# ming71/rotate-yolov3

Hardware: AMD Instinct MI355X
Metric: images/sec fwd+bwd at 608^2 (train step, backend=hip) (higher is better)
Workload: dtype bf16; 1 GPU; configs[3]: Darknet-53 train step (fwd + riou loss + bwd + grad all-reduce + SGD), bs=64/GPU 608x608, synthetic HRSC-shaped targets; global_batch=64, parallelism=dp1, gradients=250 MB fp32 in 4 flat buckets, fp32 on the wire

## Files before the change

include/ryolo.h:

```cpp
#ifndef RYOLO_H
#define RYOLO_H

#include <stddef.h>
#include <stdint.h>

#ifdef __cplusplus
extern "C" {
#endif

#define RYOLO_OK 0
#define RYOLO_EINVAL -1
#define RYOLO_ELAUNCH -2
#define RYOLO_ETOOBIG -3

#define RYOLO_RNMS_MAX_BOXES 262144

const char *ryolo_strerror(int code);
int ryolo_abi_version(void);
const char *ryolo_build_id(void);
int ryolo_set_tuning(const char *name, const char *value);

size_t ryolo_rnms_workspace_bytes(int n);
int ryolo_rnms(const float *dets, int n, int row_stride, float thr, int64_t *keep_out, int32_t *num_keep,
               void *workspace, size_t workspace_bytes, void *stream);
// ... 97 lines not shown
int ryolo_yolo_decode(const void *head, int head_cstride, int bs, int ny, int nx, int na, int no,
                      const float *anchors, float stride, float context_factor, int arc, float *io,
                      long long io_rows_per_image, long long io_row_offset, float *p, void *stream);

int ryolo_conv_head_decode_supported(const ryolo_conv_desc *desc, int na, int no);
int ryolo_conv_head_decode(const ryolo_conv_desc *desc, const void *x, const void *w_packed, const float *scale, const float *shift,
                           const float *anchors, int na, int no, float stride, float context_factor, int arc, float *io,
                           long long io_rows_per_image, long long io_row_offset, float *p, void *stream);
int ryolo_conv_head_decode_store(const ryolo_conv_desc *desc, const void *x, const void *w_packed, const float *scale, const float *shift,
                                 int na, int no, void *head, int head_cstride, float *p, void *stream);

int ryolo_add_nhwc(const void *a, int a_cstride, const void *b, int b_cstride, void *y, int y_cstride,
                   long long npix, int C, void *stream);
int ryolo_upsample_nhwc(const void *x, int x_cstride, void *y, int y_cstride, int N, int H, int W, int C, int scale,
                        void *stream);
int ryolo_maxpool_nhwc(const void *x, int x_cstride, void *y, int y_cstride, int N, int H, int W, int C, int ksize,
                       int stride, void *stream);

size_t ryolo_se_workspace_bytes(int N, int H, int W, int C);
int ryolo_se_nhwc(const void *x, int x_cstride, const float *w1 , const float *w2 ,
                  int hidden, void *y, int y_cstride, int N, int H, int W, int C,
                  float *gate_out , void *workspace, size_t workspace_bytes, void *stream);
size_t ryolo_se_bwd_workspace_bytes(int N, int H, int W, int C, int hidden);
int ryolo_se_bwd_nhwc(const void *x, int x_cstride, const void *dy, int dy_cstride, const float *w1 ,
                      const float *w2 , int hidden, void *dx , int dx_cstride, int dx_accumulate,
                      float *dw1, float *dw2 , int accumulate_w, int N, int H, int W, int C,
                      float *gate_out , void *workspace, size_t workspace_bytes, void *stream);


int ryolo_conv0_recompute_supported(const ryolo_conv_desc *desc);
int ryolo_conv0_bn_act_fwd(const ryolo_conv_desc *desc, const void *x, const void *w_packed, const float *scale, const float *shift,
                           int act, const float *slope, void *y, void *stream);
size_t ryolo_conv0_bn_bwd_workspace_bytes(void);
int ryolo_conv0_bn_bwd(const ryolo_conv_desc *desc, const void *x, const void *w_packed, const void *dy, int dy_cstride,
                       const float *scale, const float *shift, const float *mean, const float *invstd, int act, const float *slope,
                       void *dz, int dz_cstride, float *dgamma, float *dbeta, float *dslope, void *workspace, size_t workspace_bytes,
                       int workspace_is_zero, void *stream);
size_t ryolo_conv0_bn_bwd_wgrad_workspace_bytes(void);
int ryolo_conv0_bn_bwd_wgrad(const ryolo_conv_desc *desc, const void *x, const void *w_packed, const void *dy, int dy_cstride,
                             const float *scale, const float *shift, const float *mean, const float *invstd, int act, const float *slope,
                             float *dgamma, float *dbeta, float *dslope, float *grad_oihw, int cin_real, int accumulate, void *workspace,
                             size_t workspace_bytes, void *stream);
int ryolo_conv_stat_rows(const ryolo_conv_desc *desc);
int ryolo_conv2d_bn_act_stats(const ryolo_conv_desc *desc, const void *x, const void *w_packed, const float *scale,
                              const float *shift, const void *residual, void *y,
                              double *stat_part ,
                              void *stream);
int ryolo_bn_finalize(double *stat_part, int rows, int cpad, int C, long long count, float eps, float momentum,
                      const float *gamma, const float *beta, float *mean, float *invstd, float *scale, float *shift,
                      float *running_mean , float *running_var, void *stream);
int ryolo_bn_act_fwd(const void *z, int z_cstride, const float *scale, const float *shift, int act,
                     const float *slope , const void *residual, int res_cstride, void *y,
                     int y_cstride, long long npix, int C, void *stream);
size_t ryolo_bn_act_bwd_workspace_bytes(long long npix, int C);
int ryolo_bn_act_bwd(const void *z, int z_cstride, const void *dy, int dy_cstride, const float *scale, const float *shift,
                     const float *mean, const float *invstd, int act, const float *slope, void *dz, int dz_cstride,
                     long long npix, int C, float *dgamma, float *dbeta, float *dslope, void *workspace,
                     size_t workspace_bytes, void *stream);
size_t ryolo_conv_packed_dgrad_bytes(int Cout, int Cin, int ksize, int stride);
int ryolo_conv_dgrad_tap_table(int ksize, int stride, int *host_out );
int ryolo_conv_pack_weights_dgrad(const float *w_oihw, int Cout, int Cin, int ksize, int stride, void *packed,
                                  const int *taps_table ,
                                  void *stream);
int ryolo_conv2d_dgrad(const ryolo_conv_desc *forward_desc, const void *dz, int dz_cstride, const void *packed_dgrad,
                       const float *ones, const float *zeros , void *dx, int accumulate, void *stream);
int ryolo_conv2d_dgrad_bnreduce_rows(const ryolo_conv_desc *forward_desc);
int ryolo_conv2d_dgrad_bnreduce(const ryolo_conv_desc *forward_desc, const void *dz, int dz_cstride, const void *packed_dgrad,
                                const float *ones, const float *zeros, void *dx, int accumulate,
                                const void *z , int z_cstride,
                                const float *scale, const float *shift, const float *mean, const float *invstd ,
                                const float *slope , float *part , void *stream);
int ryolo_bn_act_bwd_reduced(const void *z, int z_cstride, const void *dy, int dy_cstride, const float *scale, const float *shift,
                             const float *mean, const float *invstd, int act , const float *slope, void *dz,
                             int dz_cstride, long long npix, int C, float *dgamma, float *dbeta, float *dslope, const float *part,
                             int rows, void *workspace , size_t workspace_bytes, void *stream);
size_t ryolo_conv_wgrad_workspace_bytes(const ryolo_conv_desc *forward_desc);
int ryolo_conv2d_wgrad_partials(const ryolo_conv_desc *forward_desc, const void *x, const void *dz, int dz_cstride, int Cin_real,
                                float *grad_oihw, int accumulate, void *workspace, size_t workspace_bytes, void *stream);
int ryolo_conv2d_wgrad_reduce(const ryolo_conv_desc *forward_desc, const void *x, const void *dz, int dz_cstride, int Cin_real,
                              float *grad_oihw, int accumulate, void *workspace, size_t workspace_bytes, void *stream);

typedef struct ryolo_wgrad_reduce_job {
    const float *part;
    float *g;
    int S, Cout, Cin_real, Cin_k, ks, Kpad, Cout_pad, accumulate;
    int kind;
    int block_begin, block_end;
    int wide;
} ryolo_wgrad_reduce_job;
int ryolo_conv_wgrad_reduce_job_fill(ryolo_wgrad_reduce_job *host_job, const ryolo_conv_desc *forward_desc, int Cin_real, const void *workspace,
                                     float *grad_oihw, int accumulate);
int ryolo_conv_wgrad_reduce_batch(const ryolo_wgrad_reduce_job *device_jobs, int njobs, int total_blocks, void *stream);
int ryolo_conv2d_wgrad(const ryolo_conv_desc *forward_desc, const void *x, const void *dz, int dz_cstride, int Cin_real,
                       float *grad_oihw , int accumulate, void *workspace,
                       size_t workspace_bytes, void *stream);
int ryolo_upsample2x_bwd(const void *dy, int dy_cstride, void *dx, int dx_cstride, int N, int H, int W, int C,
                         int accumulate, void *stream);
int ryolo_pgrad_to_nhwc(const float *pgrad, int bs, int na, int ny, int nx, int no, void *out, int out_cstride,
                        void *stream);

typedef struct ryolo_pack_job {
    const void *src;
    void *dst;
    int kind, Cout, Cin, KS, Cin_pad, ntaps, Kpad, rows;
    int khs[9], kws[9];
    int block_begin, block_end;
// ... 78 lines not shown
```

rotate-yolov3_amd/csrc/train.hip:

```cpp
#include "conv_common.h"

using namespace ryolo_detail;

namespace {

__global__ void __launch_bounds__(1024) bn_finalize_kernel(double *__restrict__ part, int R, int cpad, int C, float count, float eps,
                                   float momentum, const float *__restrict__ gamma, const float *__restrict__ beta,
                                   float *__restrict__ mean, float *__restrict__ invstd, float *__restrict__ scale,
                                   float *__restrict__ shift, float *__restrict__ run_mean, float *__restrict__ run_var) {
    __shared__ double red[2][32][33];
    const int cx = threadIdx.x & 31, ry = threadIdx.x >> 5;
    const int c = blockIdx.x * 32 + cx;
    double s = 0.0, q = 0.0;
    if (c < C) {
        for (int r0 = ry; r0 < R; r0 += 32 * 8) {
            double a[8], b[8];
#pragma unroll
            for (int u = 0; u < 8; u++) {
                const int r = r0 + 32 * u;
                a[u] = r < R ? part[(size_t)r * 2 * cpad + c] : 0.0;
                b[u] = r < R ? part[(size_t)r * 2 * cpad + cpad + c] : 0.0;
            }
#pragma unroll
            for (int u = 0; u < 8; u++) {
// ... 37 lines not shown
    const float n = (1.f + e) * (1.f + e);
    const float t = (n - 1.f) / (n + 1.f);
    return t + x * (1.f - t * t) * (e / (1.f + e));
}

constexpr long long NT_MIN_BYTES = 128ll << 20;
#ifdef RYOLO_MP_ABLATION
static int g_nt[3] = {-1, -1, -1};
inline bool nt_pass(int kind, long long npix, int C) { return g_nt[kind] < 0 ? npix * C * 2 >= NT_MIN_BYTES : g_nt[kind] != 0; }
#else
inline bool nt_pass(int, long long npix, int C) { return npix * C * 2 >= NT_MIN_BYTES; }
#endif
template <bool NTL>
__device__ __forceinline__ bf16x8 ld8(const __bf16 *p) {
    if constexpr (NTL) return __builtin_nontemporal_load((const bf16x8 *)p);
    else return *(const bf16x8 *)p;
}
template <bool NTL>
__device__ __forceinline__ void st8(__bf16 *p, const bf16x8 &v) {
    if constexpr (NTL) __builtin_nontemporal_store(v, (bf16x8 *)p);
    else *(bf16x8 *)p = v;
}

template <int ACT, bool NTL = false>
__global__ void bn_act_fwd_kernel(const __bf16 *__restrict__ z, int z_cs, const float *__restrict__ scale,
                                  const float *__restrict__ shift, const float *__restrict__ slope_p,
                                  const __bf16 *__restrict__ res, int res_cs, __bf16 *__restrict__ y, int y_cs,
                                  long long npix, int C) {
    const int cpr = C / 8;
    const long long total = npix * cpr;
    const float slope = slope_p ? slope_p[0] : 0.f;
    for (long long i = (long long)blockIdx.x * blockDim.x + threadIdx.x; i < total;
         i += (long long)gridDim.x * blockDim.x) {
        const long long pix = i / cpr;
        const int c = (int)(i % cpr) * 8;
        const bf16x8 v = ld8<NTL>(z + pix * z_cs + c);
        bf16x8 o;
#pragma unroll
        for (int e = 0; e < 8; e++) {
            float u = (float)v[e] * scale[c + e] + shift[c + e];
            if (ACT == 1) u = u > 0.f ? u : u * slope;
            else if (ACT == 2) u = mish_f(u);
            o[e] = (__bf16)u;
        }
        if (res) {
            const bf16x8 r = ld8<NTL>(res + pix * res_cs + c);
#pragma unroll
            for (int e = 0; e < 8; e++) o[e] = (__bf16)((float)o[e] + (float)r[e]);
        }
        st8<NTL>(y + pix * y_cs + c, o);
    }
}

constexpr int BWD_SLAB_MIN = 128;
#ifdef RYOLO_MP_ABLATION
static int g_bwd_slabs = 1024, g_bwd_slab_min = BWD_SLAB_MIN;
inline long long bwd_slab(long long npix) {
    long long s = (npix + g_bwd_slabs - 1) / g_bwd_slabs;
    return s < g_bwd_slab_min ? g_bwd_slab_min : s;
}
#else
inline long long bwd_slab(long long npix) {
    const long long s = (npix + 1023) / 1024;
    return s < BWD_SLAB_MIN ? BWD_SLAB_MIN : s;
}
#endif
template <int ACT, bool NTL = false>
__global__ void __launch_bounds__(256)
bn_act_bwd_reduce_kernel(const __bf16 *__restrict__ z, int z_cs, const __bf16 *__restrict__ dy, int dy_cs,
                         const float *__restrict__ scale, const float *__restrict__ shift,
                         const float *__restrict__ mean, const float *__restrict__ invstd,
                         const float *__restrict__ slope_p, long long npix, int C, int CT, float *__restrict__ part, long long SL) {
    __shared__ float red[256][25];
    const int cl = threadIdx.x % CT, pl = threadIdx.x / CT, npl = 256 / CT;
    const int c = (blockIdx.x * CT + cl) * 8;
    const int slab = blockIdx.y;
    const long long p0 = (long long)slab * SL;
    const long long p1 = p0 + SL < npix ? p0 + SL : npix;
    const float slope = slope_p ? slope_p[0] : 0.f;
    float s1[8], s2[8], s3[8];
#pragma unroll
    for (int e = 0; e < 8; e++) s1[e] = s2[e] = s3[e] = 0.f;
    if (c < C) {
        float sc[8], sh[8], mu[8], is[8];
#pragma unroll
        for (int e = 0; e < 8; e++) {
            sc[e] = scale ? scale[c + e] : 1.f; sh[e] = scale ? shift[c + e] : 0.f;
            mu[e] = scale ? mean[c + e] : 0.f; is[e] = scale ? invstd[c + e] : 0.f;
        }
        auto accum = [&](const bf16x8 &zv, const bf16x8 &gv) {
#pragma unroll
            for (int e = 0; e < 8; e++) {
                const float zf = (float)zv[e], d = (float)gv[e];
                float g = d;
                if (scale) {
                    const float u = zf * sc[e] + sh[e];
                    if (ACT == 1 && u <= 0.f) { g = d * slope; s3[e] += d * u; }
                    else if (ACT == 2) g = d * mish_grad(u);
                    s2[e] += g * (zf - mu[e]);
                }
                s1[e] += g;
            }
        };
        long long pix = p0 + pl;
        for (; pix + 3 * npl < p1; pix += 4 * npl) {
            bf16x8 zv[4], gv[4];
// ... 253 lines not shown
__global__ void __launch_bounds__(256) pgrad_to_nhwc_tiled_kernel(const float *__restrict__ g, int na, int plane, int no,
                                                                  __bf16 *__restrict__ out, int out_cs, int npix) {
    extern __shared__ __attribute__((aligned(16))) __bf16 pg_lds[];
    const int C = na * no;
    const int p0 = blockIdx.x * PG_PIX;
    const int per_a = PG_PIX * no;
    for (int idx = threadIdx.x; idx < na * per_a; idx += 256) {
        const int a = idx / per_a, rem = idx - a * per_a;
        const int pl = rem / no, k = rem - pl * no;
        const int gp = p0 + pl;
        if (gp < npix) {
            const int n = gp / plane, pp = gp - n * plane;
            pg_lds[pl * C + a * no + k] = (__bf16)g[((size_t)(n * na + a) * plane + pp) * no + k];
        }
    }
    __syncthreads();
    const int cpr = C / 8;
    for (int idx = threadIdx.x; idx < PG_PIX * cpr; idx += 256) {
        const int pl = idx / cpr, c = (idx - pl * cpr) * 8;
        if (p0 + pl < npix) *(bf16x8 *)(out + (size_t)(p0 + pl) * out_cs + c) = *(const bf16x8 *)(pg_lds + pl * C + c);
    }
}

constexpr int ELEM_BLOCKS = 4096;
inline int ok_launch() { return hipGetLastError() == hipSuccess ? RYOLO_OK : RYOLO_ELAUNCH; }

}

extern "C" {

int ryolo_bn_finalize(double *stat_part, int rows, int cpad, int C, long long count, float eps, float momentum,
                      const float *gamma, const float *beta, float *mean, float *invstd, float *scale, float *shift,
                      float *running_mean, float *running_var, void *stream) {
    if (!stat_part || !gamma || !beta || !mean || !invstd || !scale || !shift || rows <= 0 || C <= 0 || count <= 0)
        return RYOLO_EINVAL;
    hipLaunchKernelGGL(bn_finalize_kernel, dim3((C + 31) / 32), dim3(1024), 0, (hipStream_t)stream, stat_part, rows, cpad, C,
                       (float)count, eps, momentum, gamma, beta, mean, invstd, scale, shift, running_mean, running_var);
    return ok_launch();
}

int ryolo_bn_act_fwd(const void *z, int z_cstride, const float *scale, const float *shift, int act, const float *slope,
                     const void *residual, int res_cstride, void *y, int y_cstride, long long npix, int C, void *stream) {
    if (!z || !scale || !shift || !y || npix <= 0 || C <= 0 || (C & 7) || (z_cstride & 7) || (y_cstride & 7))
        return RYOLO_EINVAL;
    if (act < 0 || act > 2) return RYOLO_EINVAL;
    const bool ntl = nt_pass(0, npix, C);
#define RYOLO_BN_FWD(A)                                                                                                   \
    hipLaunchKernelGGL((ntl ? bn_act_fwd_kernel<A, true> : bn_act_fwd_kernel<A, false>), dim3(grid_for(npix * (C / 8))), dim3(256), 0, (hipStream_t)stream,           \
                       (const __bf16 *)z, z_cstride, scale, shift, slope, (const __bf16 *)residual, res_cstride,          \
                       (__bf16 *)y, y_cstride, npix, C)
    if (act == 0) RYOLO_BN_FWD(0); else if (act == 1) RYOLO_BN_FWD(1); else RYOLO_BN_FWD(2);
#undef RYOLO_BN_FWD
    return ok_launch();
}

size_t ryolo_bn_act_bwd_workspace_bytes(long long npix, int C) {
    const long long nslab = (npix + bwd_slab(npix) - 1) / bwd_slab(npix);
    return (size_t)nslab * 3 * C * 4 + (size_t)3 * C * 4;
}

static int bn_act_bwd_impl(const void *z, int z_cstride, const void *dy, int dy_cstride, const float *scale, const float *shift,
                           const float *mean, const float *invstd, int act, const float *slope, void *dz, int dz_cstride,
                           long long npix, int C, float *dgamma, float *dbeta, float *dslope, void *workspace,
                           size_t workspace_bytes, const float *pre_part, int pre_rows, void *stream_);

int ryolo_bn_act_bwd(const void *z, int z_cstride, const void *dy, int dy_cstride, const float *scale, const float *shift,
                     const float *mean, const float *invstd, int act, const float *slope, void *dz, int dz_cstride,
                     long long npix, int C, float *dgamma, float *dbeta, float *dslope, void *workspace,
                     size_t workspace_bytes, void *stream_) {
    return bn_act_bwd_impl(z, z_cstride, dy, dy_cstride, scale, shift, mean, invstd, act, slope, dz, dz_cstride, npix, C, dgamma, dbeta,
                           dslope, workspace, workspace_bytes, nullptr, 0, stream_);
}

int ryolo_bn_act_bwd_reduced(const void *z, int z_cstride, const void *dy, int dy_cstride, const float *scale, const float *shift,
                             const float *mean, const float *invstd, int act, const float *slope, void *dz, int dz_cstride,
                             long long npix, int C, float *dgamma, float *dbeta, float *dslope, const float *part, int rows,
                             void *workspace, size_t workspace_bytes, void *stream_) {
    if (!part || rows <= 0 || !scale || act != 1) return RYOLO_EINVAL;
    return bn_act_bwd_impl(z, z_cstride, dy, dy_cstride, scale, shift, mean, invstd, act, slope, dz, dz_cstride, npix, C, dgamma, dbeta,
                           dslope, workspace, workspace_bytes, part, rows, stream_);
}

static int bn_act_bwd_impl(const void *z, int z_cstride, const void *dy, int dy_cstride, const float *scale, const float *shift,
                           const float *mean, const float *invstd, int act, const float *slope, void *dz, int dz_cstride,
                           long long npix, int C, float *dgamma, float *dbeta, float *dslope, void *workspace,
                           size_t workspace_bytes, const float *pre_part, int pre_rows, void *stream_) {
    if (!z || !dy || npix <= 0 || C <= 0 || (C & 7) || (z_cstride & 7) || (dy_cstride & 7) || !workspace) return RYOLO_EINVAL;
    if (workspace_bytes < (pre_part ? (size_t)3 * C * 4 : ryolo_bn_act_bwd_workspace_bytes(npix, C))) return RYOLO_EINVAL;
    if (scale && (!shift || !mean || !invstd || !dz || (dz_cstride & 7))) return RYOLO_EINVAL;
    hipStream_t stream = (hipStream_t)stream_;
    int nslab = pre_part ? pre_rows : (int)((npix + bwd_slab(npix) - 1) / bwd_slab(npix));
    float *part = pre_part ? const_cast<float *>(pre_part) : (float *)workspace;
    float *s1 = pre_part ? (float *)workspace : part + (size_t)nslab * 3 * C, *s2 = s1 + C, *s3 = s2 + C;
    if (pre_part && pre_rows >= BWD_FOLD_MIN_ROWS && workspace_bytes >= (size_t)(3 + 3 * BWD_FOLD) * C * 4) {
        float *folded = s3 + C;
        const int per = (pre_rows + BWD_FOLD - 1) / BWD_FOLD;
        hipLaunchKernelGGL(bn_act_bwd_fold_kernel, dim3((C + 31) / 32, BWD_FOLD), dim3(1024), 0, stream, part, pre_rows, C, per, folded);
        part = folded;
        nslab = (pre_rows + per - 1) / per;
    }
    float *dsl = (scale && act == 1) ? dslope : nullptr;
    int CT = 32;
    while (CT > 1 && CT > C / 8) CT >>= 1;
    if (act < 0 || act > 2) return RYOLO_EINVAL;
    const bool nt_red = nt_pass(1, npix, C), nt_app = nt_pass(2, npix, C);
#define RYOLO_BN_REDK(A) (nt_red ? bn_act_bwd_reduce_kernel<A, true> : bn_act_bwd_reduce_kernel<A, false>)
// ... 84 lines not shown
```

rotate-yolov3_amd/model/hip_train_ops.py:

```python
import ctypes as C

import torch

from .. import _lib
from .._lib import PackJob, WgradReduceJob
from . import hip_ops
from .hip_ops import ConvDesc, _check_nhwc, cpad, pack_weights

ARC_FOCAL, ARC_UBCE, ARC_UCE = 1, 2, 4


def arc_flags(arc):
    f = ARC_FOCAL if 'F' in arc else 0
    if 'default' in arc:
        return f
    if 'BCE' in arc:
        return f | ARC_UBCE
    if 'CE' in arc:
        return f | ARC_UCE
    raise ValueError("unknown arc %r" % (arc,))


class WgradReduceBatch(object):

# ... 126 lines not shown


def conv0_bn_bwd_wgrad_ws(device):
    return torch.empty(_lib.lib().ryolo_conv0_bn_bwd_wgrad_workspace_bytes(), dtype=torch.uint8, device=device)


def conv0_bn_bwd_wgrad(d, x, packed_w, dy, stats, act, slope, dgamma, dbeta, dslope, grad_w, cin_real, accumulate, ws):
    mean, invstd, scale, shift = stats
    _lib.check(_lib.lib().ryolo_conv0_bn_bwd_wgrad(C.byref(d), x.data_ptr(), packed_w.data_ptr(), dy.data_ptr(), dy.stride(2),
                                                   scale.data_ptr(), shift.data_ptr(), mean.data_ptr(), invstd.data_ptr(), act,
                                                   slope.data_ptr() if slope is not None else None, dgamma.data_ptr(), dbeta.data_ptr(),
                                                   dslope.data_ptr() if dslope is not None else None, grad_w.data_ptr(), int(cin_real),
                                                   1 if accumulate else 0, ws.data_ptr(), ws.numel(), _s(x.device)), "ryolo_conv0_bn_bwd_wgrad")


def conv_fwd_plain(d, x, packed_w, ones, shift, z):
    d.out_cstride = _check_nhwc(z, "z")
    _lib.check(_lib.lib().ryolo_conv2d_bn_act(C.byref(d), x.data_ptr(), packed_w.data_ptr(), ones.data_ptr(), shift.data_ptr(),
                                              None, z.data_ptr(), _s(x.device)), "ryolo_conv2d_bn_act")


def conv_head_decode_store(hf, x, packed_w, ones, shift, head, p):
    d = ConvDesc(*hf['desc'])
    d.in_cstride = _check_nhwc(x, "x")
    hcs = _check_nhwc(head, "head")
    if not p.is_contiguous() or p.dtype != torch.float32:
        raise ValueError("conv_head_decode_store: p must be contiguous fp32")
    _lib.check(_lib.lib().ryolo_conv_head_decode_store(C.byref(d), x.data_ptr(), packed_w.data_ptr(), ones.data_ptr(), shift.data_ptr(),
                                                       hf['na'], hf['no'], head.data_ptr(), hcs, p.data_ptr(), _s(x.device)),
               "ryolo_conv_head_decode_store")


def bn_finalize(part, C_, count, gamma, beta, eps=1e-5, momentum=0.1, running_mean=None, running_var=None, out=None):
    dev = part.device
    if out is None:
        out = [torch.empty(C_, dtype=torch.float32, device=dev) for _ in range(4)]
    _lib.check(_lib.lib().ryolo_bn_finalize(part.data_ptr(), part.shape[0], part.shape[2], C_, int(count), eps, momentum,
                                            gamma.data_ptr(), beta.data_ptr(), out[0].data_ptr(), out[1].data_ptr(),
                                            out[2].data_ptr(), out[3].data_ptr(),
                                            running_mean.data_ptr() if running_mean is not None else None,
                                            running_var.data_ptr() if running_var is not None else None, _s(dev)),
               "ryolo_bn_finalize")
    return out


def bn_act_fwd(z, scale, shift, act, slope, y, residual=None):
    n, h, w, c = z.shape
    _lib.check(_lib.lib().ryolo_bn_act_fwd(z.data_ptr(), z.stride(2), scale.data_ptr(), shift.data_ptr(), act,
                                           slope.data_ptr() if slope is not None else None,
                                           residual.data_ptr() if residual is not None else None,
                                           residual.stride(2) if residual is not None else 0, y.data_ptr(), y.stride(2),
                                           n * h * w, c, _s(z.device)), "ryolo_bn_act_fwd")
    return y


def bn_act_bwd(z, dy, stats, act, slope, dz, dgamma, dbeta, dslope, ws):
    n, h, w, c = z.shape
    mean, invstd, scale, shift = stats if stats is not None else (None, None, None, None)
    p = lambda t: t.data_ptr() if t is not None else None
    _lib.check(_lib.lib().ryolo_bn_act_bwd(z.data_ptr(), z.stride(2), dy.data_ptr(), dy.stride(2), p(scale), p(shift), p(mean),
                                           p(invstd), act, p(slope), p(dz), dz.stride(2) if dz is not None else 0,
                                           n * h * w, c, p(dgamma), p(dbeta), p(dslope), ws.data_ptr(), ws.numel(),
                                           _s(z.device)), "ryolo_bn_act_bwd")


def bn_bwd_ws_bytes(npix, c):
    return _lib.lib().ryolo_bn_act_bwd_workspace_bytes(npix, c)


_tap_tables = {}


def dgrad_tap_table(ksize, stride, device):
    key = (ksize, stride, device.index)
    t = _tap_tables.get(key)
    if t is None:
        host = (C.c_int * 72)()
        _lib.check(_lib.lib().ryolo_conv_dgrad_tap_table(ksize, stride, host), "ryolo_conv_dgrad_tap_table")
        t = torch.tensor(list(host), dtype=torch.int32, device=device)
        _tap_tables[key] = t
    return t


def pack_weights_dgrad(weight, stride, out=None):
    cout, cin, k, _ = weight.shape
    L = _lib.lib()
    nbytes = L.ryolo_conv_packed_dgrad_bytes(cout, cin, k, stride)
    if out is None:
        out = torch.empty(nbytes, dtype=torch.uint8, device=weight.device)
    w = weight.contiguous()
    table = dgrad_tap_table(k, stride, weight.device)
    _lib.check(L.ryolo_conv_pack_weights_dgrad(w.data_ptr(), cout, cin, k, stride, out.data_ptr(), table.data_ptr(),
                                               _s(weight.device)), "ryolo_conv_pack_weights_dgrad")
    return out


def conv_dgrad(d, dz, packed_dgrad, ones, zeros, dx, accumulate):
    _lib.check(_lib.lib().ryolo_conv2d_dgrad(C.byref(d), dz.data_ptr(), dz.stride(2), packed_dgrad.data_ptr(), ones.data_ptr(),
                                             zeros.data_ptr(), dx.data_ptr(), 1 if accumulate else 0, _s(dz.device)),
               "ryolo_conv2d_dgrad")


def dgrad_bnreduce_rows(d):
    return _lib.lib().ryolo_conv2d_dgrad_bnreduce_rows(C.byref(d))


# ... 338 lines not shown
```

rotate-yolov3_amd/model/plan.py:

```python
import ctypes as C
from collections import namedtuple

from .. import _lib
from .._lib import ACT_LINEAR, ConvDesc

View = namedtuple('View', 'buf off C H W cs')
EvalPlan = namedtuple('EvalPlan', 'shapes buffers x views ops')
CONV_TYPES = ('convolutional', 'd-convolutional')
TrainPlan = namedtuple('TrainPlan', 'shapes buffers x act grd forward blocks backward')


class Refused(RuntimeError):
    """the configuration is refused at plan time (as opposed to a bug in the planner)"""


def _abs(i, l):
    return l if l > 0 else i + l


def _sources(i, d):
    return [_abs(i, int(v)) for v in d['layers'].split(',')]


def shared_attrs(d):
# ... 304 lines not shown
            recompute = bool(i == 0 and cv['bn'] and i not in conv_res and conv0_recompute
                             and _query('ryolo_conv0_recompute_supported', desc))
            head_fused = None
            if (head_decode and yolos is not None and i + 1 < n and defs[i + 1]['type'] == 'yolo' and readers[i] == [i + 1] and i not in home
                    and i not in conv_res and not cv['bn'] and cv['k'] == 1 and cv['s'] == 1 and c % 8 == 0):
                na, no = yolos[i + 1]
                ht = (N, xin.H, xin.W, xin.C, c, 1, 1, 0, xin.cs, c, 0, ACT_LINEAR, 0.0, 1, 0)
                if _query('ryolo_conv_head_decode_supported', ht, int(na), int(no)):
                    head_fused = dict(desc=ht, na=int(na), no=int(no))
            blk = dict(layer=i, desc=desc, xin=xin, xin_g=xin_g, y=y, dy=dy, res=act[conv_res[i]] if i in conv_res else None,
                       res_g=grd[conv_res[i]] if i in conv_res else None, res_alias=res_alias, bn=cv['bn'], act=cv['act'], shape=shp[i],
                       recompute=recompute, one_pass=bool(recompute and xin_g is None and conv0_one_pass), head_fused=head_fused)
            blocks.append(blk)
            forward.append(('conv', i, blk))
        elif t == 'shortcut':
            a, b = i - 1, _abs(i, int(d['from']))
            act[i], grd[i] = pair_for(i)
            forward.append(('add', i, (act[a], act[b], act[i], grd[a], grd[b], grd[i])))
        elif t == 'upsample':
            act[i], grd[i] = pair_for(i)
            forward.append(('up', i, (act[i - 1], act[i], grd[i - 1], grd[i])))
        elif t == 'route':
            if i in alias:
                act[i], grd[i] = act[alias[i]], grd[alias[i]]
        elif t == 'yolo':
            act[i], grd[i] = act[i - 1], grd[i - 1]
            forward.append(('yolo', i, (act[i], grd[i])))

    init = set()

    def first(g):
        if g in init:
            return False
        init.add(g)
        init.update(children.get(g, ()))
        return True

    heads = [i for kind, i, _ in forward if kind == 'yolo']
    backward = []
    for kind, i, pl in reversed(forward):
        if kind == 'yolo':
            first(pl[1])
            backward.append((kind, i, heads.index(i)))
        elif kind == 'conv':
            res_first = first(pl['res_g']) if (pl['res_g'] is not None and not pl['res_alias']) else None
            backward.append((kind, i, (res_first, first(pl['xin_g']) if pl['xin_g'] is not None else None)))
        elif kind == 'add':
            backward.append((kind, i, (first(pl[3]), first(pl[4]))))
        elif kind == 'up':
            backward.append((kind, i, first(pl[2])))
    return TrainPlan(shp, buffers, x, act, grd, forward, blocks, backward)


def reduce_fusion_pairs(tp):
    by = {b['layer']: b for b in tp.blocks}
    pairs = []
    for (k0, i0, _), (k1, i1, _) in zip(tp.backward[:-1], tp.backward[1:]):
        if k0 != 'conv' or k1 != 'conv':
            continue
        x, y = by[i0], by[i1]
        g, dy = x['xin_g'], y['dy']
        if g is None or not y['bn'] or y['recompute'] or g != dy or dy[2:5] != y['shape'] or g.cs != g.C:
            continue
        rows = _query('ryolo_conv2d_dgrad_bnreduce_rows', x['desc'])
        if rows > 0:
            pairs.append((x, y, rows))
    return pairs
```

rotate-yolov3_amd/model/train_engine.py:

```python
import ctypes as C
import os

import torch
import torch.nn as nn

from .. import _lib
from . import hip_ops as ops
from . import hip_train_ops as tr
from . import plan
from .engine import HipEngine
from .nhwc_batch import NHWC8Batch


class _Fn(torch.autograd.Function):
    @staticmethod
    def forward(ctx, engine, x, anchor):
        ctx.engine = engine
        outs = engine.forward(x)
        return tuple(outs)

    @staticmethod
    def backward(ctx, *grads):
        ctx.engine.backward(grads)
        return None, None, None
# ... 63 lines not shown
                    dz = None if rec['one_pass'] else new_buf(c, h, w)
                else:
                    z, dz = y, dy
                blk = dict(i=i, conv=conv, bn=bn, act=actmod[-1] if actmod else None, mish=any(type(s_).__name__ == 'Mish' for s_ in mods[i]),
                           xin=xin, xin_g=tv(rec['xin_g']), z=z, dz=dz, y=y, dy=dy, desc=desc, res=tv(rec['res']), res_g=tv(rec['res_g']),
                           res_alias=rec['res_alias'], cin_k=xin.shape[-1], k=desc.ksize, s=desc.stride, pad=desc.pad,
                           npix=self.bs * h * w, C=c, recompute=rec['recompute'])
                if rec.get('head_fused') and not actmod and not blk['mish']:
                    blk['head_fused'] = rec['head_fused']
                wgrad_ws = max(wgrad_ws, tr.wgrad_ws_bytes(desc))
                bn_ws = max(bn_ws, tr.bn_bwd_ws_bytes(blk['npix'], c))
                self.blocks.append(blk)
                fwd.append(('conv', i, blk))
            elif kind in ('add', 'up'):
                fwd.append((kind, i, tuple(tv(v) for v in rec)))
            elif kind == 'yolo':
                m = mods[i]
                c, h, w = tp.shapes[i]
                anchors = m.anchors.to(device=device, dtype=torch.float32).contiguous()
                pbuf = torch.empty((self.bs, m.na, h, w, model.nc + 6), dtype=torch.float32, device=device)
                io = None
                if model.nc + 6 > 96 or m.na * (model.nc + 6) > 1024:
                    io = torch.empty((self.bs, m.na * h * w, model.nc + 6), dtype=torch.float32, device=device)
                self.p.append(pbuf)
                hb = self.blocks[-1] if self.blocks and self.blocks[-1]['i'] == i - 1 and self.blocks[-1].get('head_fused') else None
                if hb is not None and (hb['head_fused']['na'], hb['head_fused']['no']) != (m.na, model.nc + 6):
                    hb.pop('head_fused')
                    hb = None
                fwd.append(('yolo', i, (tv(rec[0]), tv(rec[1]), m, anchors, pbuf, io, h, w, hb)))
        self.head_pairs = [(pl[0], pl[1]) for kind, _, pl in fwd if kind == 'yolo']
        self.fused_nhwc = False
        self.head_g_ready = False
        self.head_bias_fold = os.environ.get('RYOLO_HEAD_BIAS_FOLD', '1') != '0'
        self.head_gscale = torch.ones(1, device=device)
        self.head_bias_ready = None
        self._bias_parts = self._bias_ws = None
        self._fold_now = (False,) * len(self.head_pairs)
        self._g_bwd_fold = None
        readers = plan._readers(defs)
        for k, (hd, _) in enumerate(self.head_pairs):
            for b in self.blocks:
                i = b['i']
                if (b['y'] is hd and b['bn'] is None and b['conv'].bias is not None and i + 1 < len(defs) and defs[i + 1]['type'] == 'yolo'
                        and readers[i] == [i + 1]):
                    b['head_k'] = k
        self.batch_reduce = os.environ.get('RYOLO_WGRAD_BATCH_REDUCE', '1') != '0'
        self._wr_batches = {}
        self._ws_w_bytes = max(wgrad_ws, 256)
        self._ws_w = None
        self.ws_b = torch.empty(max(bn_ws, 256), dtype=torch.uint8, device=device)

        self.bplan = [(kind, i, pl, flags) for (kind, i, pl), (_, _, flags) in zip(reversed(fwd), tp.backward)]

    @staticmethod
    def _conv_attrs(m):
        conv = HipEngine._conv_of(m)
        other = [type(s_).__name__ for s_ in m if not isinstance(s_, (nn.Conv2d, nn.BatchNorm2d, nn.PReLU, nn.LeakyReLU))
                 and type(s_).__name__ != 'Mish']
        return dict(cout=conv.out_channels, k=conv.kernel_size[0], s=conv.stride[0], pad=conv.padding[0],
                    bn=HipEngine._bn_of(m) is not None, act=None,
                    refuse="activation %s has no HIP training kernels (use model.backend = 'torch')" % other[0] if other else None)

    def _build_grad_sink(self):
        plist = [q for q in self.model.parameters()]
        views = getattr(self.model, '_dp_grad_views', None)
        ok = views is not None and os.environ.get("RYOLO_DIRECT_GRADS", "1") != "0"
        if ok:
            for q in plist:
                v = views.get(q)
                if (v is None or v.dtype != torch.float32 or not v.is_contiguous() or v.device != q.device or v.shape != q.shape
                        or q.grad is None or q.grad.data_ptr() != v.data_ptr()):
                    ok = False
                    break
        self.direct = bool(ok)
        if ok:
            self.static_flat = None
            self.static_grad = {q: views[q] for q in plist}
        else:
            self.static_flat = torch.zeros(sum(q.numel() for q in plist), dtype=torch.float32, device=self.device)
            off = 0
            for q in plist:
                self.static_grad[q] = self.static_flat[off:off + q.numel()].view_as(q)
                off += q.numel()

    def _reset_grad_sink(self):
        self.static_grad, self.static_flat, self.direct = {}, None, False
        self._segs, self.g_bwd = None, None
        self._wr_batches = {}

    def _check_direct_sink(self):
        if not self.direct:
            return
        rebound = 0
        for q, v in self.static_grad.items():
            g = q.grad
            if g is None:
                v.zero_()
            elif g.data_ptr() != v.data_ptr():
                v.copy_(g)
            else:
                continue
            q.grad = v
            rebound += 1
        if rebound and not getattr(self, '_warned_rebind', False):
            self._warned_rebind = True
            import warnings
# ... 131 lines not shown
                if self.g_fwd is None:
                    self.g_fwd = self._capture(self._forward_launch)
                if self.g_fwd is not None:
                    self.g_fwd.replay()
        return [p for p in self.p]

    def _capture(self, launch):
        dev = self.device
        torch.cuda.synchronize(dev)
        g = torch.cuda.CUDAGraph()
        try:
            with torch.cuda.graph(g, capture_error_mode="thread_local"):
                launch()
            return g
        except Exception as e:
            self.use_graph = False
            self.graph_fallback = "%s: %s" % (type(e).__name__, str(e).splitlines()[0][:200] if str(e) else "")
            import warnings
            warnings.warn("TrainEngine: hipGraph capture failed (%s); continuing with eager launches" % self.graph_fallback)
            try:
                torch.cuda.synchronize(dev)
            except Exception:
                pass
            launch()
            return None

    def _forward_launch(self):
        dev = self.device
        L = _lib.lib()
        if self.nbt is None:
            self.nbt = [pl['bn'].num_batches_tracked for kind, i, pl in self.plan if kind == 'conv' and pl['bn'] is not None]
        if self.nbt:
            torch._foreach_add_(self.nbt, 1)
        if self.packs is None:
            self.packs = tr.WeightPackBatch(dev)
            for kind, i, pl in self.plan:
                if kind != 'conv':
                    continue
                w = pl['conv'].weight
                if w.dtype != torch.float32 or not w.is_contiguous():
                    raise RuntimeError("TrainEngine expects contiguous fp32 conv weights")
                cout, cin, k, _ = w.shape
                pl['packed'] = torch.empty(L.ryolo_conv_packed_weight_bytes(cout, pl['cin_k'], k), dtype=torch.uint8, device=dev)
                pl['packed_d'] = torch.empty(L.ryolo_conv_packed_dgrad_bytes(cout, cin, k, pl['s']), dtype=torch.uint8,
                                             device=dev) if pl['xin_g'] is not None else None
                self.packs.add(w.detach(), pl['s'], pl['cin_k'], pl['packed'], pl['packed_d'])
            self.packs.finalize()
        self.packs.run()
        for kind, i, pl in self.plan:
            if kind == 'conv':
                b = pl
                conv, bn = b['conv'], b['bn']
                if bn is not None:
                    part = tr.conv_fwd_stats(b['desc'], b['xin'], b['packed'], self.ones, self.zeros, b['z'], part=self.stat_part,
                                             clear=False)
                    b['stats'] = tr.bn_finalize(part, b['C'], b['npix'], bn.weight.detach(), bn.bias.detach(), eps=bn.eps,
                                                momentum=bn.momentum, running_mean=bn.running_mean,
                                                running_var=bn.running_var, out=b.get('stats'))
                    slope = b['act'].weight.detach() if isinstance(b['act'], nn.PReLU) else None
                    if isinstance(b['act'], nn.LeakyReLU):
                        if 'leaky' not in b:
                            b['leaky'] = torch.full((1,), b['act'].negative_slope, device=dev)
                        slope = b['leaky']
                    b['slope'] = slope
                    b['actcode'] = 2 if b['mish'] else (1 if slope is not None else 0)
                    if b['recompute']:
                        tr.conv0_bn_act_fwd(b['desc'], b['xin'], b['packed'], b['stats'][2], b['stats'][3], b['actcode'], slope, b['y'])
                    else:
                        tr.bn_act_fwd(b['z'], b['stats'][2], b['stats'][3], b['actcode'], slope, b['y'], residual=b['res'])
                else:
                    if conv.bias is not None:
                        if 'bias_pad' not in b:
                            b['bias_pad'] = torch.zeros(ops.cpad(b['C']), device=dev)
                        b['bias_pad'][:b['C']].copy_(conv.bias.detach())
                        bias = b['bias_pad']
                    else:
                        bias = self.zeros
                    b['bias_now'] = bias
                    if not b.get('head_fused'):
                        tr.conv_fwd_plain(b['desc'], b['xin'], b['packed'], self.ones, bias, b['z'])
                    b['stats'] = None
            elif kind == 'add':
                a, bb, y = pl[0], pl[1], pl[2]
                nn_, hh, ww, cc = y.shape
                _lib.check(L.ryolo_add_nhwc(a.data_ptr(), a.stride(2), bb.data_ptr(), bb.stride(2), y.data_ptr(), y.stride(2),
                                            nn_ * hh * ww, cc, _lib.stream_ptr(dev)), "ryolo_add_nhwc")
            elif kind == 'up':
                xin, y = pl[0], pl[1]
                nn_, hh, ww, cc = xin.shape
                _lib.check(L.ryolo_upsample_nhwc(xin.data_ptr(), xin.stride(2), y.data_ptr(), y.stride(2), nn_, hh, ww, cc, 2,
                                                 _lib.stream_ptr(dev)), "ryolo_upsample_nhwc")
            elif kind == 'yolo':
                head, _, m, anchors, pbuf, io, hh, ww, hb = pl
                stride = float(max(self.H, self.W)) / float(max(hh, ww))
                if hb is not None:
                    tr.conv_head_decode_store(hb['head_fused'], hb['xin'], hb['packed'], self.ones, hb['bias_now'], head, pbuf)
                else:
                    _lib.check(L.ryolo_yolo_decode(head.data_ptr(), head.stride(2), self.bs, hh, ww, m.na, self.model.nc + 6,
                                                   anchors.data_ptr(), stride, 1.0, 0, io.data_ptr() if io is not None else None, m.na * hh * ww, 0,
                                                   pbuf.data_ptr(), _lib.stream_ptr(dev)), "ryolo_yolo_decode")
                if (m.nx, m.ny) != (ww, hh):
                    from .models import create_grids
                    create_grids(m, (self.H, self.W), (ww, hh), dev)

    def backward(self, pgrads):
        dev = self.device
        with torch.cuda.device(dev), torch.no_grad():
            if not hasattr(self, "static_pg"):
                self.static_pg = [torch.zeros_like(p) for p in self.p]
            ready, bias_ready = self.head_g_ready, self.head_bias_ready
            self.head_g_ready, self.head_bias_ready = False, None
            fold = [False] * len(self.static_pg)
            for k, (buf, g) in enumerate(zip(self.static_pg, pgrads)):
                if g is not None and ready and g.data_ptr() == buf.data_ptr():
                    fold[k] = bias_ready is not None and bias_ready[k] is not None
                    continue
                if g is None:
                    buf.zero_()
                elif g.data_ptr() != buf.data_ptr():
                    buf.copy_(g)
# ... 134 lines not shown
```

Measured before the change: 1377 images/s.

## Fuse BN+activation(+residual) forward with the following 1x1 conv and its BN statistics

Adds a persistent kernel that applies BN scale/shift, leaky/PReLU and an optional residual to z, writes y, stages the tile in LDS, and immediately runs the next 1x1 conv (C to C/2) with MFMA. It also accumulates that conv's BN sum and sum-of-squares into stat_part. The engine pairs eligible bn->1x1 conv layers for channel classes 64, 128 and 512, skipping the separate conv_fwd_stats launch and the re-read of y. The cost is more complex register and LDS use, weights held in registers, and a different precision path for the stats, since they are computed from bf16-rounded outputs.

```diff
diff --git a/include/ryolo.h b/include/ryolo.h
--- a/include/ryolo.h
+++ b/include/ryolo.h
@@ -173,6 +173,10 @@
 int ryolo_bn_act_fwd(const void *z, int z_cstride, const float *scale, const float *shift, int act,
                      const float *slope , const void *residual, int res_cstride, void *y,
                      int y_cstride, long long npix, int C, void *stream);
+int ryolo_bn_act_conv1x1_stats_supported(const ryolo_conv_desc *next_1x1, int C, int has_res);
+int ryolo_bn_act_conv1x1_stats(const ryolo_conv_desc *next_1x1, const void *z, int z_cs, const float *scale, const float *shift,
+                               const float *slope, const void *res, int res_cs, void *y, int y_cs, const void *packed_w, void *z2,
+                               int z2_cs, double *stat_part, long long npix, void *stream);
 size_t ryolo_bn_act_bwd_workspace_bytes(long long npix, int C);
 int ryolo_bn_act_bwd(const void *z, int z_cstride, const void *dy, int dy_cstride, const float *scale, const float *shift,
                      const float *mean, const float *invstd, int act, const float *slope, void *dz, int dz_cstride,
diff --git a/rotate-yolov3_amd/csrc/train.hip b/rotate-yolov3_amd/csrc/train.hip
--- a/rotate-yolov3_amd/csrc/train.hip
+++ b/rotate-yolov3_amd/csrc/train.hip
@@ -113,6 +113,207 @@
     }
 }
 
+template <int KT, int WN, int WM, int PF, bool HAS_RES, bool NTL>
+__global__ void __launch_bounds__(WN * WM * 64)
+bn_act_pw_kernel(const __bf16 *__restrict__ z, int z_cs, const float *__restrict__ scale, const float *__restrict__ shift,
+                 const float *__restrict__ slope_p, const __bf16 *__restrict__ res, int res_cs, __bf16 *__restrict__ y, int y_cs,
+                 const __bf16 *__restrict__ w, __bf16 *__restrict__ z2, int z2_cs, int nt_z2, double *__restrict__ stat_part,
+                 int stat_cpad, long long npix, long long nblk) {
+    constexpr int CF = 2;
+    constexpr int C = KT * 64, COUT = WN * CF * 16, BM = WM * PF * 16, NTHR = WN * WM * 64;
+    constexpr int CPR = C / 8;
+    constexpr int RPP = NTHR / CPR;
+    constexpr int NCH = BM / RPP;
+    constexpr int UNIT = BM * 128;
+    static_assert(NTHR % CPR == 0 && BM % RPP == 0 && NCH >= 1, "the threads must tile a row block");
+    static_assert(2 * 2 * COUT * 4 * WM <= KT * UNIT, "the statistics fold reuses the tile");
+    extern __shared__ __attribute__((aligned(16))) char smem[];
+
+    const int tid = threadIdx.x, lane = tid & 63;
+    const int wave = __builtin_amdgcn_readfirstlane(tid >> 6);
+    const int fr = lane & 15, g = lane >> 4;
+    const int wn = wave % WN, wm = wave / WN;
+
+    const int cslot = tid % CPR, r0 = tid / CPR;
+    const int c = cslot * 8;
+    const float slope = slope_p ? slope_p[0] : 0.f;
+    int lds_wr[NCH];
+#pragma unroll
+    for (int j = 0; j < NCH; j++) {
+        const int row = r0 + j * RPP;
+        lds_wr[j] = (cslot >> 3) * UNIT + row * 128 + (((cslot & 7) ^ ((row >> 1) & 7)) << 4);
+    }
+    bf16x8 zv[NCH], rv[HAS_RES ? NCH : 1];
+    auto request = [&](int j, long long blk) __attribute__((always_inline)) {
+        long long m = blk * BM + r0 + j * RPP;
+        m = m < npix ? m : npix - 1;
+        zv[j] = ld8<NTL>(z + m * z_cs + c);
+        if constexpr (HAS_RES) rv[j] = ld8<NTL>(res + m * res_cs + c);
+    };
+    long long blk = blockIdx.x;
+#pragma unroll
+    for (int j = 0; j < NCH; j++) request(j, blk);
+    float sc[8], sh[8];
+#pragma unroll
+    for (int e = 0; e < 8; e++) {
+        sc[e] = scale[c + e];
+        sh[e] = shift[c + e];
+    }
+
+    bf16x8 wreg[KT][2][CF];
+#pragma unroll
+    for (int kt = 0; kt < KT; kt++)
+#pragma unroll
+        for (int ks = 0; ks < 2; ks++)
+#pragma unroll
+            for (int cf = 0; cf < CF; cf++)
+                wreg[kt][ks][cf] = *(const bf16x8 *)(w + (size_t)(wn * CF * 16 + cf * 16 + fr) * C + kt * 64 + ks * 32 + g * 8);
+    int a_rd[2];
+#pragma unroll
+    for (int ks = 0; ks < 2; ks++) a_rd[ks] = (wm * PF * 16 + fr) * 128 + (((ks * 4 + g) ^ ((fr >> 1) & 7)) << 4);
+    const int och = wn * CF * 16 + (g & 1) * 16 + (g >> 1) * 8;
+    float st_sum[CF][4], st_sq[CF][4];
+#pragma unroll
+    for (int cf = 0; cf < CF; cf++)
+#pragma unroll
+        for (int rr = 0; rr < 4; rr++) st_sum[cf][rr] = st_sq[cf][rr] = 0.f;
+
+    for (; blk < nblk; blk += gridDim.x) {
+#pragma unroll
+        for (int j = 0; j < NCH; j++) {
+            const long long m = blk * BM + r0 + j * RPP;
+            const bool ok = m < npix;
+            const bf16x8 v = zv[j];
+            bf16x8 o;
+#pragma unroll
+            for (int e = 0; e < 8; e++) {
+                float u = (float)v[e] * sc[e] + sh[e];
+                u = u > 0.f ? u : u * slope;
+                o[e] = (__bf16)u;
+            }
+            if constexpr (HAS_RES) {
+                const bf16x8 r = rv[j];
+#pragma unroll
+                for (int e = 0; e < 8; e++) o[e] = (__bf16)((float)o[e] + (float)r[e]);
+            }
+            request(j, blk + gridDim.x);
+            if (ok) {
+                st8<NTL>(y + m * y_cs + c, o);
+            } else {
+#pragma unroll
+                for (int e = 0; e < 8; e++) o[e] = (__bf16)0.f;
+            }
+            *(bf16x8 *)(smem + lds_wr[j]) = o;
+        }
+        __syncthreads();
+
+        f32x4 acc[CF][PF];
+#pragma unroll
+        for (int cf = 0; cf < CF; cf++)
+#pragma unroll
+            for (int f = 0; f < PF; f++) acc[cf][f] = f32x4{0.f, 0.f, 0.f, 0.f};
+#pragma unroll
+        for (int kt = 0; kt < KT; kt++)
+#pragma unroll
+            for (int ks = 0; ks < 2; ks++) {
+                bf16x8 xf[PF];
+#pragma unroll
+                for (int f = 0; f < PF; f++) xf[f] = *(const bf16x8 *)(smem + kt * UNIT + a_rd[ks] + f * 2048);
+#pragma unroll
+                for (int cf = 0; cf < CF; cf++)
+#pragma unroll
+                    for (int f = 0; f < PF; f++)
+                        acc[cf][f] = __builtin_amdgcn_mfma_f32_16x16x32_bf16(wreg[kt][ks][cf], xf[f], acc[cf][f], 0, 0, 0);
+            }
+        __syncthreads();
+
+        const long long m0 = blk * BM + wm * PF * 16;
+#pragma unroll
+        for (int f = 0; f < PF; f++) {
+            unsigned R[CF][2];
+#pragma unroll
+            for (int cf = 0; cf < CF; cf++) {
+                bf16x4 o;
+#pragma unroll
+                for (int rr = 0; rr < 4; rr++) {
+                    o[rr] = (__bf16)acc[cf][f][rr];
+                    const float qv = (float)o[rr];
+                    st_sum[cf][rr] += qv;
+                    st_sq[cf][rr] += qv * qv;
+                }
+                const uint2 u2 = __builtin_bit_cast(uint2, o);
+                R[cf][0] = u2.x;
+                R[cf][1] = u2.y;
+            }
+#if defined(__HIP_DEVICE_COMPILE__)
+            auto s0 = __builtin_amdgcn_permlane16_swap(R[0][0], R[1][0], false, false);
+            auto s1 = __builtin_amdgcn_permlane16_swap(R[0][1], R[1][1], false, false);
+            const bf16x8 out = __builtin_bit_cast(bf16x8, u32x4{s0[0], s1[0], s0[1], s1[1]});
+            const long long m = m0 + f * 16 + fr;
+            if (m < npix) {
+                if (nt_z2) st8<true>(z2 + m * z2_cs + och, out);
+                else st8<false>(z2 + m * z2_cs + och, out);
+            }
+#endif
+        }
+    }
+
+    float ta = 0.f, tb = 0.f;
+#pragma unroll
+    for (int cf = 0; cf < CF; cf++)
+#pragma unroll
+        for (int rr = 0; rr < 4; rr++) {
+            const float a = row16_sum(st_sum[cf][rr]), b = row16_sum(st_sq[cf][rr]);
+            if (fr == cf * 4 + rr) {
+                ta = a;
+                tb = b;
+            }
+        }
+    float *red = (float *)smem;
+    if (fr < CF * 4) {
+        const int ch = wn * CF * 16 + (fr >> 2) * 16 + g * 4 + (fr & 3);
+        red[(wm * 2 + 0) * COUT + ch] = ta;
+        red[(wm * 2 + 1) * COUT + ch] = tb;
+    }
+    __syncthreads();
+    for (int t = tid; t < 2 * COUT; t += NTHR) {
+        float v = 0.f;
+#pragma unroll
+        for (int k = 0; k < WM; k++) v += red[k * 2 * COUT + t];
+        double *row = stat_part + (size_t)(blockIdx.x % STAT_ROWS) * 2 * stat_cpad;
+        atomicAdd(row + (t / COUT) * stat_cpad + (t % COUT), (double)v);
+    }
+}
+
+template <int KT, int WN, int WM, int PF>
+int bn_pw_launch(const void *z, int z_cs, const float *scale, const float *shift, const float *slope, const void *res, int res_cs, void *y,
+                 int y_cs, const void *w, void *z2, int z2_cs, double *stat_part, int stat_cpad, long long npix, hipStream_t stream) {
+    constexpr int C = KT * 64, BM = WM * PF * 16, NTHR = WN * WM * 64, LDS = KT * BM * 128;
+    const bool ntl = nt_pass(0, npix, C);
+    const int nt_z2 = npix * (C / 2) * 2 >= NT_OUT_MIN_BYTES ? 1 : 0;
+    const long long nblk = (npix + BM - 1) / BM;
+    long long grid = cu_count();
+    if (grid > nblk) grid = nblk;
+#define RYOLO_BN_PW(R, N)                                                                                                            \
+    return launch_kernel<bn_act_pw_kernel<KT, WN, WM, PF, R, N>>(dim3((unsigned)grid), dim3(NTHR), LDS, stream, (const __bf16 *)z, z_cs, \
+                                                                 scale, shift, slope, (const __bf16 *)res, res_cs, (__bf16 *)y, y_cs,  \
+                                                                 (const __bf16 *)w, (__bf16 *)z2, z2_cs, nt_z2, stat_part, stat_cpad,  \
+                                                                 npix, nblk)
+    if (res) {
+        if (ntl) RYOLO_BN_PW(true, true);
+        RYOLO_BN_PW(true, false);
+    }
+    if (ntl) RYOLO_BN_PW(false, true);
+    RYOLO_BN_PW(false, false);
+#undef RYOLO_BN_PW
+}
+
+inline bool bn_pw_shape(const ryolo_conv_desc *d, int C) {
+    if (!d || d->ksize != 1 || d->stride != 1 || d->pad != 0 || d->upsample != 1 || d->N <= 0 || d->H <= 0 || d->W <= 0) return false;
+    if (d->Cin != C || d->Cout * 2 != C) return false;
+    return C == 64 || C == 128 || C == 256 || C == 512;
+}
+
 constexpr int BWD_SLAB_MIN = 128;
 #ifdef RYOLO_MP_ABLATION
 static int g_bwd_slabs = 1024, g_bwd_slab_min = BWD_SLAB_MIN;
@@ -472,6 +673,27 @@
     if (act == 0) RYOLO_BN_FWD(0); else if (act == 1) RYOLO_BN_FWD(1); else RYOLO_BN_FWD(2);
 #undef RYOLO_BN_FWD
     return ok_launch();
+}
+
+int ryolo_bn_act_conv1x1_stats_supported(const ryolo_conv_desc *next_1x1, int C, int has_res) {
+    (void)has_res;
+    return bn_pw_shape(next_1x1, C) ? 1 : 0;
+}
+
+int ryolo_bn_act_conv1x1_stats(const ryolo_conv_desc *next_1x1, const void *z, int z_cs, const float *scale, const float *shift,
+                               const float *slope, const void *res, int res_cs, void *y, int y_cs, const void *packed_w, void *z2, int z2_cs,
+                               double *stat_part, long long npix, void *stream) {
+    if (!next_1x1 || !z || !scale || !shift || !y || !packed_w || !z2 || !stat_part || npix <= 0) return RYOLO_EINVAL;
+    const int C = next_1x1->Cin;
+    if (!bn_pw_shape(next_1x1, C) || npix != (long long)next_1x1->N * next_1x1->H * next_1x1->W) return RYOLO_EINVAL;
+    if ((z_cs & 7) || (y_cs & 7) || (z2_cs & 7) || z_cs < C || y_cs < C || z2_cs < C / 2 || (res && ((res_cs & 7) || res_cs < C))) return RYOLO_EINVAL;
+    if ((((uintptr_t)z | (uintptr_t)y | (uintptr_t)z2 | (uintptr_t)res | (uintptr_t)packed_w) & 15)) return RYOLO_EINVAL;
+    const int cpad = (C / 2 + 127) / 128 * 128;
+    hipStream_t s = (hipStream_t)stream;
+    if (C == 64) return bn_pw_launch<1, 1, 8, 1>(z, z_cs, scale, shift, slope, res, res_cs, y, y_cs, packed_w, z2, z2_cs, stat_part, cpad, npix, s);
+    if (C == 128) return bn_pw_launch<2, 2, 4, 2>(z, z_cs, scale, shift, slope, res, res_cs, y, y_cs, packed_w, z2, z2_cs, stat_part, cpad, npix, s);
+    if (C == 256) return bn_pw_launch<4, 4, 2, 2>(z, z_cs, scale, shift, slope, res, res_cs, y, y_cs, packed_w, z2, z2_cs, stat_part, cpad, npix, s);
+    return bn_pw_launch<8, 8, 1, 2>(z, z_cs, scale, shift, slope, res, res_cs, y, y_cs, packed_w, z2, z2_cs, stat_part, cpad, npix, s);
 }
 
 size_t ryolo_bn_act_bwd_workspace_bytes(long long npix, int C) {
diff --git a/rotate-yolov3_amd/model/hip_train_ops.py b/rotate-yolov3_amd/model/hip_train_ops.py
--- a/rotate-yolov3_amd/model/hip_train_ops.py
+++ b/rotate-yolov3_amd/model/hip_train_ops.py
@@ -202,6 +202,25 @@
                                            residual.stride(2) if residual is not None else 0, y.data_ptr(), y.stride(2),
                                            n * h * w, c, _s(z.device)), "ryolo_bn_act_fwd")
     return y
+
+
+def bn_act_conv1x1_stats_supported(d, c, has_res):
+    return bool(_lib.lib().ryolo_bn_act_conv1x1_stats_supported(C.byref(d), int(c), 1 if has_res else 0))
+
+
+def bn_act_conv1x1_stats(d, z, scale, shift, slope, y, residual, packed_w, z2, part):
+    n, h, w, c = z.shape
+    rows, cp = stat_rows(), cpad(d.Cout)
+    part = part.view(-1)[:rows * 2 * cp].view(rows, 2, cp)
+    _check_nhwc(y, "y")
+    _check_nhwc(z2, "z2")
+    _lib.check(_lib.lib().ryolo_bn_act_conv1x1_stats(C.byref(d), z.data_ptr(), z.stride(2), scale.data_ptr(), shift.data_ptr(),
+                                                     slope.data_ptr() if slope is not None else None,
+                                                     residual.data_ptr() if residual is not None else None,
+                                                     residual.stride(2) if residual is not None else 0, y.data_ptr(), y.stride(2),
+                                                     packed_w.data_ptr(), z2.data_ptr(), z2.stride(2), part.data_ptr(), n * h * w,
+                                                     _s(z.device)), "ryolo_bn_act_conv1x1_stats")
+    return part
 
 
 def bn_act_bwd(z, dy, stats, act, slope, dz, dgamma, dbeta, dslope, ws):
diff --git a/rotate-yolov3_amd/model/plan.py b/rotate-yolov3_amd/model/plan.py
--- a/rotate-yolov3_amd/model/plan.py
+++ b/rotate-yolov3_amd/model/plan.py
@@ -380,6 +380,21 @@
     return TrainPlan(shp, buffers, x, act, grd, forward, blocks, backward)
 
 
+def fwd_bn_pw_pairs(tp):
+    pairs = []
+    for (k0, _, y), (k1, _, x) in zip(tp.forward[:-1], tp.forward[1:]):
+        if k0 != 'conv' or k1 != 'conv':
+            continue
+        if not y['bn'] or y['recompute'] or y.get('head_fused') or not x['bn'] or x['recompute']:
+            continue
+        d = x['desc']
+        if d[5] != 1 or d[6] != 1 or d[7] != 0 or x['xin'] != y['y']:
+            continue
+        if _query('ryolo_bn_act_conv1x1_stats_supported', d, int(y['shape'][0]), 1 if y['res'] is not None else 0):
+            pairs.append((y, x))
+    return pairs
+
+
 def reduce_fusion_pairs(tp):
     by = {b['layer']: b for b in tp.blocks}
     pairs = []
diff --git a/rotate-yolov3_amd/model/train_engine.py b/rotate-yolov3_amd/model/train_engine.py
--- a/rotate-yolov3_amd/model/train_engine.py
+++ b/rotate-yolov3_amd/model/train_engine.py
@@ -139,6 +139,21 @@
 
         self.bplan = [(kind, i, pl, flags) for (kind, i, pl), (_, _, flags) in zip(reversed(fwd), tp.backward)]
 
+        self.fwd_pw_pairs = []
+        sw = os.environ.get('RYOLO_FWD_BN_PW', '1')
+        if sw != '0':
+            classes = None if sw == 'all' else (self.FWD_PW_CLASSES if sw == '1' else tuple(int(v) for v in sw.split(',')))
+            by = {b['i']: b for b in self.blocks}
+            for yr, xr in plan.fwd_bn_pw_pairs(tp):
+                yb, xb = by[yr['layer']], by[xr['layer']]
+                if classes is not None and yb['C'] not in classes:
+                    continue
+                if isinstance(yb['act'], (nn.PReLU, nn.LeakyReLU)) and not yb['mish']:
+                    yb['pw_next'], xb['pw_prev'] = xb, yb
+                    self.fwd_pw_pairs.append((yb['i'], xb['i']))
+
+    FWD_PW_CLASSES = (64, 128, 512)
+
     @staticmethod
     def _conv_attrs(m):
         conv = HipEngine._conv_of(m)
@@ -376,8 +391,11 @@
                 b = pl
                 conv, bn = b['conv'], b['bn']
                 if bn is not None:
-                    part = tr.conv_fwd_stats(b['desc'], b['xin'], b['packed'], self.ones, self.zeros, b['z'], part=self.stat_part,
-                                             clear=False)
+                    if b.get('pw_prev') is not None:
+                        part = b['pw_prev']['pw_part']
+                    else:
+                        part = tr.conv_fwd_stats(b['desc'], b['xin'], b['packed'], self.ones, self.zeros, b['z'], part=self.stat_part,
+                                                 clear=False)
                     b['stats'] = tr.bn_finalize(part, b['C'], b['npix'], bn.weight.detach(), bn.bias.detach(), eps=bn.eps,
                                                 momentum=bn.momentum, running_mean=bn.running_mean,
                                                 running_var=bn.running_var, out=b.get('stats'))
@@ -390,6 +408,10 @@
                     b['actcode'] = 2 if b['mish'] else (1 if slope is not None else 0)
                     if b['recompute']:
                         tr.conv0_bn_act_fwd(b['desc'], b['xin'], b['packed'], b['stats'][2], b['stats'][3], b['actcode'], slope, b['y'])
+                    elif b.get('pw_next') is not None:
+                        nx = b['pw_next']
+                        b['pw_part'] = tr.bn_act_conv1x1_stats(nx['desc'], b['z'], b['stats'][2], b['stats'][3], slope, b['y'], b['res'],
+                                                               nx['packed'], nx['z'], self.stat_part)
                     else:
                         tr.bn_act_fwd(b['z'], b['stats'][2], b['stats'][3], b['actcode'], slope, b['y'], residual=b['res'])
                 else:
```

New measurement: 1389 images/s (median of 6 runs). About the same (+0.9%).
